# BlackCloud37/rust-raytracer

Hardware: AMD Instinct MI355X
Metric: Msamples/sec (px*spp), scene_500 1200x1200 1000spp (higher is better)
Workload: dtype f64

## Files before the change

### rust-raytracer_amd/csrc/abi.cpp

```cpp
#include <algorithm>
#include <cmath>
#include <cstdlib>
#include <cstring>
#include <functional>
#include <mutex>
#include <new>
#include <string>
#include <vector>

#include "common/grid_shape.h"
#include "common/rng.h"
#include "common/schedule.h"
#include "device/adaptive.h"
#include "device/ao.h"
#include "device/denoise.h"
#include "device/device.h"
#include "host/frame.h"
#include "host/scene.h"
#include "rtamd.h"

using namespace rtamd;

static thread_local std::string g_err;
static Tuning g_tuning;
// ... 951 lines not shown
}

int rt_tonemap_u8(const double* rgb, size_t n_channels, uint8_t* out) {
    return guard([&] {
        REQUIRE((rgb && out) || n_channels == 0, "null argument");
        for (size_t i = 0; i < n_channels; i++) out[i] = tonemap_channel(rgb[i]);
        return (int)RT_OK;
    });
}
int rt_write_png(const char* path, int width, int height, const uint8_t* rgb) {
    return guard([&] {
        REQUIRE(path, "null path");
        write_png(path, width, height, rgb);
        return (int)RT_OK;
    });
}

int rt_debug_rng_device(uint64_t seed, uint64_t pixel, uint64_t sample, int n, uint64_t* out_host) {
    return guard([&] {
        REQUIRE(n > 0 && out_host, "bad argument");
        if (device_count() < 1) throw RtError(RT_ERR_NO_DEVICE, "no HIP device");
        debug_rng_device(seed, pixel, sample, n, out_host);
        return (int)RT_OK;
    });
}
int rt_debug_rng_host(uint64_t seed, uint64_t pixel, uint64_t sample, int n, uint64_t* out_host) {
    return guard([&] {
        REQUIRE(n > 0 && out_host, "bad argument");
        Rng r;
        r.seed_stream(seed, pixel, sample);
        for (int i = 0; i < n; i++) out_host[i] = r.next_u64();
        return (int)RT_OK;
    });
}
int rt_debug_rng_floats(uint64_t seed, uint64_t pixel, uint64_t sample, int n, double lo, double hi, int on_device, double* out_gen,
                        double* out_range) {
    return guard([&] {
        REQUIRE(n > 0 && out_gen && out_range && lo < hi && std::isfinite(hi - lo), "bad argument");
        if (on_device) {
            if (device_count() < 1) throw RtError(RT_ERR_NO_DEVICE, "no HIP device");
            debug_rng_floats_device(seed, pixel, sample, n, lo, hi, out_gen, out_range);
            return (int)RT_OK;
        }
        Rng r;
        r.seed_stream(seed, pixel, sample);
        for (int i = 0; i < n; i++) out_gen[i] = r.gen_f64();
        r.seed_stream(seed, pixel, sample);
        for (int i = 0; i < n; i++) out_range[i] = (lo == -1. && hi == 1.) ? r.gen_range_pm1() : (lo == 0. && hi == 1.) ? r.gen_range_01() : r.gen_range(lo, hi);
        return (int)RT_OK;
    });
}
int rt_debug_math_device(int op, size_t n, const double* a_host, const double* b_host, double* out_host) {
    return guard([&] {
        REQUIRE(n > 0 && a_host && out_host && (op == 0 || op == 2 || op == 3 || (op == 1 && b_host)), "bad argument");
        if (device_count() < 1) throw RtError(RT_ERR_NO_DEVICE, "no HIP device");
        debug_math_device(op, n, a_host, b_host, out_host);
        return (int)RT_OK;
    });
}
int rt_debug_hit_device(const rt_scene* s, int kernel, size_t n, const double* rays_host, double t_min, double t_max, double* out_host) {
    return guard([&] {
        REQUIRE(s && n > 0 && rays_host && out_host && (kernel == 1 || kernel == 2 || kernel == 3 || kernel == 5 || kernel == 6 || kernel == 7), "bad argument");
        if (device_count() < 1) throw RtError(RT_ERR_NO_DEVICE, "no HIP device");
        debug_hit_device(*s, kernel, n, rays_host, t_min, t_max, out_host);
        return (int)RT_OK;
    });
}
static int env_debug(const rt_scene* s, int device, const std::function<void()>& f) {
    return guard([&] {
        REQUIRE(s, "null scene");
        const int n_dev = device_count();
        if (n_dev < 1 || !env_debug_linked()) throw RtError(RT_ERR_NO_DEVICE, "no HIP device");
        REQUIRE(device >= 0 && device < n_dev, "no such device");
        DeviceScope dev_scope(device);
        f();
        return (int)RT_OK;
    });
}
int rt_debug_env_table_device(const rt_scene* s, int device, int* w, int* h, uint32_t* q_host) {
    return env_debug(s, device, [&] { debug_env_table_device(*s, w, h, q_host); });
}
int rt_debug_env_sample_device(const rt_scene* s, int device, size_t n, const double* xi4_host, double* out_host) {
    return env_debug(s, device, [&] {
        REQUIRE(n > 0 && xi4_host && out_host, "bad argument");
        debug_env_eval_device(*s, 0, n, xi4_host, out_host);
    });
}
int rt_debug_env_pdf_device(const rt_scene* s, int device, size_t n, const double* dirs_host, double* pdf_host) {
    return env_debug(s, device, [&] {
        REQUIRE(n > 0 && dirs_host && pdf_host, "bad argument");
        debug_env_eval_device(*s, 1, n, dirs_host, pdf_host);
    });
}
int rt_debug_area_sample_device(const rt_scene* s, int device, size_t n, const double* in_host, double* out_host) {
    return env_debug(s, device, [&] {
        REQUIRE(n > 0 && in_host && out_host, "bad argument");
        if (&rtamd::debug_area_eval_device == nullptr) throw RtError(RT_ERR_NO_DEVICE, "no HIP device");
        debug_area_eval_device(*s, 0, n, in_host, out_host);
    });
}
int rt_debug_area_pdf_device(const rt_scene* s, int device, size_t n, const double* rays_host, double* pdf_host) {
    return env_debug(s, device, [&] {
        REQUIRE(n > 0 && rays_host && pdf_host, "bad argument");
        if (&rtamd::debug_area_eval_device == nullptr) throw RtError(RT_ERR_NO_DEVICE, "no HIP device");
        debug_area_eval_device(*s, 1, n, rays_host, pdf_host);
    });
}
// ... 154 lines not shown
```

### rust-raytracer_amd/csrc/device/kernels.hip

```cpp
#include <hip/hip_runtime.h>

#include <cmath>
#include <cstdio>
#include <chrono>
#include <cstdlib>
#include <cstring>
#include <map>
#include <memory>
#include <mutex>
#include <vector>

#include "../common/flat.h"
#include "../common/grid_shape.h"
#include "../common/detlog.h"
#include "../common/detsin.h"
#include "../common/detuv.h"
#include "../common/rng.h"
#include "../common/schedule.h"
#include "../common/tighten.h"
#include "device.h"

namespace rtamd {

#ifndef PT_BLOCK
// ... 61 lines not shown
DEV double dot(D3 a, D3 b) { return a.x * b.x + a.y * b.y + a.z * b.z; }
DEV double sqlen(D3 a) { return a.x * a.x + a.y * a.y + a.z * a.z; }
DEV D3 cross(D3 a, D3 b) { return mk(a.y * b.z - a.z * b.y, a.z * b.x - a.x * b.z, a.x * b.y - a.y * b.x); }
DEV double comp(D3 a, int i) { return i == 0 ? a.x : (i == 1 ? a.y : a.z); }
DEV D3 unit(D3 a, int* err) {
    double l = sqrt(sqlen(a));
    if (l == 0.) atomicOr(err, 1);
    return divs(a, l);
}
DEV bool near_zero(D3 a) {
    const double S = 1e-8;
    return (fabs(a.x) < S) && (fabs(a.y) < S) && (fabs(a.z) < S);
}
DEV D3 reflect(D3 v, D3 n) { return sub(v, muls(n, 2. * dot(v, n))); }
DEV D3 refract(D3 uv, D3 n, double eta) {
    double cos_theta = fmin(dot(neg(uv), n), 1.0);
    D3 perp = muls(add(uv, muls(n, cos_theta)), eta);
    D3 par = muls(n, -sqrt(fabs(1.0 - sqlen(perp))));
    return add(perp, par);
}
DEV D3 random_in_unit_sphere(Rng& rng) {
    double u, v, r2;
    for (;;) {
        u = rng.gen_range_pm1();
        v = rng.gen_range_pm1();
        r2 = u * u + v * v;
        if (r2 <= 1.) break;
    }
    double q = sqrt(1. - r2);
    return mk(2. * u * q, 2. * v * q, 1. - 2. * r2);
}
DEV D3 random_in_unit_disk(Rng& rng) {
    for (;;) {
        double a = rng.gen_range_pm1();
        double b = rng.gen_range_pm1();
        if (a * a + b * b + 0. * 0. >= 1.) continue;
        return mk(a, b, 0.);
    }
}
DEV D3 xf_point(const double* t, D3 p) {
    return mk(t[0] * p.x + t[1] * p.y + t[2] * p.z + t[3] * 1., t[4] * p.x + t[5] * p.y + t[6] * p.z + t[7] * 1.,
              t[8] * p.x + t[9] * p.y + t[10] * p.z + t[11] * 1.);
}
DEV D3 xf_dir(const double* t, D3 p) {
    return mk(t[0] * p.x + t[1] * p.y + t[2] * p.z + t[3] * 0., t[4] * p.x + t[5] * p.y + t[6] * p.z + t[7] * 0.,
              t[8] * p.x + t[9] * p.y + t[10] * p.z + t[11] * 0.);
}

#define AS_G __attribute__((address_space(1)))
#define AS_L __attribute__((address_space(3)))
typedef unsigned int u32x4 __attribute__((ext_vector_type(4)));
typedef float f32x4 __attribute__((ext_vector_type(4)));
typedef float f32x2 __attribute__((ext_vector_type(2)));
struct Acc {
    const uint2* meta;
    const double2* boxes;
    const double2* spheres;
    const int* sphere_mat;
    const double2* rects;
    const int* rect_mat;
    const uint4* tris;
    const double2* tripre;
    const double2* tripre2;
    const AS_L f32x4* n2_top;
    uint32_t n2_top_count;
    uint32_t n2w_lds;
    const double* xforms;
    const MatDev* mats;
    const TexDev* texs;
    const double* vpos;
    const double* vnrm;
    const uint8_t* texels;
    uint32_t n_nodes;
    const float4* n2;
    const uint2* items2;
    const uint2* inst2;
    uint32_t root2;
    const uint2* lights;
    uint32_t n_lights;
    const MediumDev* media;
    const double* msph;
    const uint32_t* tie_view;
    uint32_t time_lds;
    const uint4* n2q;
    const uint4* n2q_top;
    uint32_t n2q_top_count;
    const uint4* tri32;
    const double* qgrid;
};
template <class P>
DEV Acc make_acc(P hot, const char* gbase, const FlatView& v) {
    Acc a;
    a.meta = (const uint2*)(hot + v.off_meta);
    a.boxes = (const double2*)(hot + v.off_boxes);
    a.spheres = (const double2*)(hot + v.off_spheres);
    a.rects = (const double2*)(hot + v.off_rects);
    a.tris = (const uint4*)(hot + v.off_tris);
    a.tripre = (const double2*)(hot + v.off_tripre);
    a.tripre2 = (const double2*)(hot + v.off_tripre2);
    a.n2_top = nullptr;
    a.n2_top_count = 0;
    a.n2w_lds = 0;
    a.xforms = (const double*)(hot + v.off_xforms);
    a.vpos = (const double*)(gbase + v.off_vpos);
    a.sphere_mat = (const int*)(gbase + v.off_sphere_mat);
    a.rect_mat = (const int*)(gbase + v.off_rect_mat);
    a.mats = (const MatDev*)(gbase + v.off_mats);
    a.texs = (const TexDev*)(gbase + v.off_texs);
    a.vnrm = (const double*)(gbase + v.off_vnrm);
    a.texels = (const uint8_t*)(gbase + v.off_texels);
    a.n_nodes = v.n_nodes;
    a.n2 = (const float4*)(hot + v.off_n2);
    a.items2 = (const uint2*)(hot + v.off_items2);
    a.inst2 = (const uint2*)(hot + v.off_inst2);
    a.root2 = v.root2;
    a.lights = (const uint2*)(gbase + v.off_lights);
    a.n_lights = v.n_lights;
    a.media = (const MediumDev*)(gbase + v.off_media);
    a.msph = (const double*)(gbase + v.off_msph);
    a.tie_view = (const uint32_t*)(gbase + v.off_tie_view);
    a.time_lds = 0u;
    return a;
}

struct CamK {
    D3 origin, llc, horizontal, vertical, u, v;
    double lens_radius;
};
struct RenderK {
    int width, height, max_depth;
    double t_min;
    uint64_t seed;
    int s_begin, s_end;
    int sub_spp, subs_per_tile, n_units;
    int tiles_x, rank, world;
    int tiles_owned;
    int job_units;
    int lvl[5][5];
    int pool_mode;
    const double* sppm_est;
    int n_top;
    int n_topq;
    int coop_pool;
    int coop_stack;
    double time0, time1;
    int time_slots;
    const int* tile_list;
    float box_shrink;
};

DEV bool aabb_hit(const double2* b, D3 o, D3 inv, double t_min, double t_max) {
    double2 v0 = b[0], v1 = b[1], v2 = b[2];
    double mn = t_min, mx = t_max;
    {
        double t0 = (v0.x - o.x) * inv.x, t1 = (v1.y - o.x) * inv.x;
        if (inv.x < 0.0) { double s = t0; t0 = t1; t1 = s; }
        mn = fmax(mn, t0);
        mx = fmin(mx, t1);
    }
    {
        double t0 = (v0.y - o.y) * inv.y, t1 = (v2.x - o.y) * inv.y;
        if (inv.y < 0.0) { double s = t0; t0 = t1; t1 = s; }
        mn = fmax(mn, t0);
        mx = fmin(mx, t1);
    }
    {
        double t0 = (v1.x - o.z) * inv.z, t1 = (v2.y - o.z) * inv.z;
        if (inv.z < 0.0) { double s = t0; t0 = t1; t1 = s; }
        mn = fmax(mn, t0);
        mx = fmin(mx, t1);
    }
    return !(mx <= mn);
}
#ifndef RT_SPHERE_F32_REJECT
#define RT_SPHERE_F32_REJECT 0
#endif
DEV bool sphere_hit(const double2* s, D3 o, D3 d, double a, double t_min, double t_max, double& t_out) {
    double2 c0 = s[0], c1 = s[1];
    D3 oc = mk(o.x - c0.x, o.y - c0.y, o.z - c1.x);
    double radius = c1.y;
    if (RT_SPHERE_F32_REJECT) {
        const float x = (float)oc.x, y = (float)oc.y, z = (float)oc.z, dx = (float)d.x, dy = (float)d.y, dz = (float)d.z, r32 = (float)radius;
        const float hb = __builtin_fmaf(z, dz, __builtin_fmaf(y, dy, x * dx));
        const float a32 = __builtin_fmaf(dz, dz, __builtin_fmaf(dy, dy, dx * dx));
        const float c32 = __builtin_fmaf(z, z, __builtin_fmaf(y, y, x * x)) - r32 * r32;
        const float disc32 = __builtin_fmaf(hb, hb, -(a32 * c32));
        const float m = fmaxf(fmaxf(fabsf(x), fabsf(y)), fabsf(z)) + fabsf(r32), dm = fmaxf(fmaxf(fabsf(dx), fabsf(dy)), fabsf(dz));
        const float bound = 7.62939453125e-06f * (dm * m) * (dm * m);
        if (disc32 < -bound) return false;
    }
    double half_b = dot(oc, d);
    double c = sqlen(oc) - radius * radius;
    double disc = half_b * half_b - a * c;
    if (disc < 0.) return false;
    double sq = sqrt(disc);
    double root = (-half_b - sq) / a;
    if (!(root >= t_min && root <= t_max)) root = (-half_b + sq) / a;
    if (!(root >= t_min && root <= t_max)) return false;
    t_out = root;
    return true;
}
DEV bool rect_hit(const double2* r, int axis, D3 o, D3 d, double t_min, double t_max, double& t_out) {
    double2 r0 = r[0], r1 = r[1], r2 = r[2];
    double t = (r2.x - comp(o, axis)) / comp(d, axis);
    if (t < t_min || t > t_max) return false;
    D3 p = add(o, muls(d, t));
    double a, b;
    if (axis == 2) { a = p.x; b = p.y; }
    else if (axis == 1) { a = p.x; b = p.z; }
    else { a = p.y; b = p.z; }
    if (a < r0.x || a > r1.x || b < r0.y || b > r1.y) return false;
    t_out = t;
    return true;
}
DEV double ray_time(const Acc& A) { return A.time_lds ? *(const AS_L double*)(uintptr_t)(A.time_lds + 8u * threadIdx.x) : 0.; }
DEV D3 msphere_center(const double* q, double time) {
    const D3 c0 = mk(q[0], q[1], q[2]), c1 = mk(q[3], q[4], q[5]);
    return add(c0, muls(sub(c1, c0), (time - q[6]) / (q[7] - q[6])));
}
__device__ __attribute__((noinline)) bool msphere_hit(const double* q, double time, double ox, double oy, double oz, double dx, double dy, double dz, double a,
                                                       double t_min, double t_max, double* t_out) {
    const D3 c = msphere_center(q, time), o = mk(ox, oy, oz), d = mk(dx, dy, dz);
    const D3 oc = sub(o, c);
    const double radius = q[8];
    const double half_b = dot(oc, d);
    const double cc = sqlen(oc) - radius * radius;
    const double disc = half_b * half_b - a * cc;
    if (disc < 0.) return false;
    const double sq = sqrt(disc);
    double root = (-half_b - sq) / a;
    if (!(root >= t_min && root <= t_max)) root = (-half_b + sq) / a;
    if (!(root >= t_min && root <= t_max)) return false;
    *t_out = root;
    return true;
}
DEV int perlin_cell(double fx) {
    const double m = fx - 256. * floor(fx * 0.00390625);
    return (m >= 0. && m < 256.) ? (int)m : 0;
}
__device__ __attribute__((noinline)) double noise_marble(const uint8_t* tab, double scale, double px, double py, double pz) {
    const double* ranvec = (const double*)tab;
    const uint8_t* perm = tab + 768 * sizeof(double);
    double accum_t = 0., weight = 1.;
    double x = px, y = py, z = pz;
    const double NEAR = 33554432.;
    const bool near = (fabs(px) < NEAR) && (fabs(py) < NEAR) && (fabs(pz) < NEAR);
    for (int oct = 0; oct < 7; oct++) {
        const double fx = floor(x), fy = floor(y), fz = floor(z);
        const double u = x - fx, v = y - fy, w = z - fz;
        int i, j, k;
        if (near) {
            i = (int)fx; j = (int)fy; k = (int)fz;
        } else {
// ... 346 lines not shown
    const float tf = fminf(fminf(qx, qy), qz);
    entry = tn;
    float m;
    asm("v_min_f32 %0, %1, %2" : "=v"(m) : "v"(tf), "v"(r.best));
    return !(tn > m) && !(r.tmin > tf);
}
DEV bool box32s(float nx, float ny, float nz, float fx, float fy, float fz, const Ray32& r, float& entry) {
    const float px = __builtin_fmaf(nx, r.ix, -r.cx), qx = __builtin_fmaf(fx, r.ix, -r.cx);
    const float py = __builtin_fmaf(ny, r.iy, -r.cy), qy = __builtin_fmaf(fy, r.iy, -r.cy);
    const float pz = __builtin_fmaf(nz, r.iz, -r.cz), qz = __builtin_fmaf(fz, r.iz, -r.cz);
    const float tn = fmaxf(fmaxf(px, py), pz);
    const float tf = fminf(fminf(qx, qy), qz) * (1.0f + 9.5367431640625e-7f);
    entry = tn;
    return !(tn > tf) && !(tn > r.best) && !(r.tmin > tf);
}
struct SignMasks {
    uint64_t x, y, z;
};
DEV SignMasks sign_masks(const Ray32& r) {
    SignMasks m;
    m.x = __ballot(r.ix < 0.f);
    m.y = __ballot(r.iy < 0.f);
    m.z = __ballot(r.iz < 0.f);
    return m;
}
DEV uint32_t sel32(uint32_t if_clear, uint32_t if_set, uint64_t lane_mask) {
    uint32_t v;
    asm("v_cndmask_b32_e64 %0, %1, %2, %3" : "=v"(v) : "v"(if_clear), "v"(if_set), "s"(lane_mask));
    return v;
}
DEV bool box32(float lox, float loy, float loz, float hix, float hiy, float hiz, const Ray32& r, float& entry) {
    float px = __builtin_fmaf(lox, r.ix, -r.cx), qx = __builtin_fmaf(hix, r.ix, -r.cx);
    float py = __builtin_fmaf(loy, r.iy, -r.cy), qy = __builtin_fmaf(hiy, r.iy, -r.cy);
    float pz = __builtin_fmaf(loz, r.iz, -r.cz), qz = __builtin_fmaf(hiz, r.iz, -r.cz);
    float tn = fmaxf(fmaxf(fminf(px, qx), fminf(py, qy)), fminf(pz, qz));
    float tf = fminf(fminf(fmaxf(px, qx), fmaxf(py, qy)), fmaxf(pz, qz)) * (1.0f + 9.5367431640625e-7f);
    entry = tn;
    return !(tn > tf) && !(tn > r.best) && !(r.tmin > tf);
}

__host__ __device__ inline size_t walk_stack_bytes(uint32_t rows, uint32_t threads) { return (size_t)rows * threads * sizeof(uint32_t); }
__host__ __device__ inline uint32_t coop_stack_rows(const FlatView& v) {
    const uint32_t d = (v.world_depth2 > v.inst_depth2 ? v.world_depth2 : v.inst_depth2) + 2u;
    return d > v.stack2_inline ? d : v.stack2_inline;
}
struct MediaTrack {
    uint32_t lim[2];
    double exitt[2];
    double T[2];
};
DEV double track_bound(const MediaTrack& K, double best) {
    return fmax(best, fmax(K.lim[0] != 0u ? fmin(K.T[0], K.exitt[0]) : 0., K.lim[1] != 0u ? fmin(K.T[1], K.exitt[1]) : 0.));
}
template <int GENERAL, bool DEFER = false, bool TOP = true, bool WIDE = false, class PEND = uint32_t, bool LIMIT = false, bool ENTER = !DEFER, bool TRACK = false, bool RESOLVE = true,
          bool TIEDEF = false>
DEV Hit traverse2(const Acc& A, uint32_t* stk, const int stride, D3 wo, D3 wd, double t_min, double t_max, PEND* pend = nullptr, uint32_t order_limit = 0xFFFFFFFFu,
                  MediaTrack* track = nullptr) {
    D3 o = wo, d = wd;
    Hit h;
    h.t = t_max;
    h.node = -1;
    h.xf = -1;
    h.kp = 0;
    int cur_xf = -1;
    double a = sqlen(d);
    constexpr bool TIE = TIE_RULE && GENERAL != 0 && (!DEFER || TIEDEF) && !LIMIT && !(TRACK && RT_TIE_NOTRACK);
    Ray32 r = make_ray32(o, d, t_min, t_max);
    float best_all32 = r.best;
    if (WIDE) ray32_wide_addr(r, A.n2w_lds);
    int sp = 0;
    const uint32_t spw_step = 4u * (uint32_t)stride;
    uint32_t spw = WIDE ? (uint32_t)(uintptr_t)(AS_L uint32_t*)stk + spw_step : 0u;
    if (WIDE) *(AS_L uint32_t*)stk = REF_DONE;
    uint32_t cur = WIDE ? wide_ref(A.root2) : A.root2;
    for (;;) {
        while ((cur >> REF_TAG_SHIFT) == 0u) {
            PH_EV(10);
#ifdef RTAMD_PHASE_STATS
            if (GENERAL && cur_xf >= 0) PH_EV(15);
#endif
            if (WIDE) {
                const uint32_t axx = cur + r.ax, ayy = cur + r.ay, azz = cur + r.az;
                f32x2 nx, fx, ny, fy, nz, fz, cc;
                asm volatile(
                    "ds_read_b64 %0, %7\n\t"
                    "ds_read_b64 %1, %7 offset:%10\n\t"
                    "ds_read_b64 %2, %8\n\t"
                    "ds_read_b64 %3, %8 offset:%10\n\t"
                    "ds_read_b64 %4, %9\n\t"
                    "ds_read_b64 %5, %9 offset:%10\n\t"
                    "ds_read_b64 %6, %7 offset:24\n\t"
                    "s_waitcnt lgkmcnt(0)"
                    : "=&v"(nx), "=&v"(fx), "=&v"(ny), "=&v"(fy), "=&v"(nz), "=&v"(fz), "=&v"(cc)
                    : "v"(axx), "v"(ayy), "v"(azz), "n"(NODEW_FAR)
                    : "memory");
                float e0, e1;
                const bool h0 = box32w(nx.x, ny.x, nz.x, fx.x, fy.x, fz.x, r, e0);
                const bool h1 = box32w(nx.y, ny.y, nz.y, fx.y, fy.y, fz.y, r, e1);
                const uint32_t c0 = __float_as_uint(cc.x), c1 = __float_as_uint(cc.y);
                if (h0 && h1) {
                    const bool swap = e1 < e0;
                    *(AS_L uint32_t*)(uintptr_t)spw = swap ? c0 : c1;
                    spw += spw_step;
                    cur = swap ? c1 : c0;
                } else if (h0) {
                    cur = c0;
                } else if (h1) {
                    cur = c1;
// ... 1 lines not shown
                    spw -= spw_step;
                    cur = *(const AS_L uint32_t*)(uintptr_t)spw;
                }
                continue;
            }
            f32x4 q0, q1, q2;
            f32x2 q3;
            f32x2 q3m = {0.f, 0.f};
            if (TOP && cur < A.n2_top_count) {
                const AS_L f32x4* p = A.n2_top + NODE2_F4 * cur;
                q0 = p[0]; q1 = p[1]; q2 = p[2]; q3 = *(const AS_L f32x2*)(p + 3);
                if (LIMIT || TRACK) q3m = ((const AS_L f32x2*)(p + 3))[1];
            } else {
                const f32x4* p = (const f32x4*)A.n2 + NODE2_F4 * cur;
                q0 = p[0]; q1 = p[1]; q2 = p[2]; q3 = *(const f32x2*)(p + 3);
                if (LIMIT || TRACK) q3m = ((const f32x2*)(p + 3))[1];
            }
            float e0, e1;
            bool h0 = box32(q0.x, q0.z, q1.x, q1.z, q2.x, q2.z, r, e0);
            bool h1 = box32(q0.y, q0.w, q1.y, q1.w, q2.y, q2.w, r, e1);
            if (LIMIT) {
                h0 = h0 && __float_as_uint(q3m.x) < order_limit;
                h1 = h1 && __float_as_uint(q3m.y) < order_limit;
            }
            if (TRACK) {
                const uint32_t lim = max(track->lim[0], track->lim[1]);
                h0 = h0 && (__float_as_uint(q3m.x) < lim || !(e0 > best_all32));
                h1 = h1 && (__float_as_uint(q3m.y) < lim || !(e1 > best_all32));
            }
            uint32_t c0 = __float_as_uint(q3.x), c1 = __float_as_uint(q3.y);
            if (h0 && h1) {
                bool swap = e1 < e0;
                uint32_t nearc = swap ? c1 : c0, farc = swap ? c0 : c1;
                stk[sp] = farc;
                sp += stride;
                cur = nearc;
            } else if (h0) {
                cur = c0;
            } else if (h1) {
                cur = c1;
            } else if (sp > 0) {
                sp -= stride;
                cur = stk[sp];
            } else {
                cur = REF_DONE;
            }
        }
        if (!WIDE && cur == REF_DONE) break;
        PH_BEGIN(ph_leaf0);
        if (WIDE && cur == REF_DONE) {
        } else if ((cur >> REF_TAG_SHIFT) == 1u) {
            uint32_t first = cur & REF_LEAF_FIRST_MASK, cnt = ((cur >> REF_LEAF_COUNT_SHIFT) & 7u) + 1u;
            uint32_t enter = REF_DONE;
            for (uint32_t i = 0; i < cnt; i++) {
                PH_EV(11);
                uint2 it = A.items2[first + i];
                uint32_t kind = it.x & NK_MASK, pl = it.x >> NK_BITS;
                double t = 0.;
                bool got = false;
                uint32_t cube_side = 0u;
                const double t_far = TRACK ? track_bound(*track, TIE ? h.t * TIE_W : h.t) : (TIE ? h.t * TIE_W : h.t);
                if (LIMIT && it.y >= order_limit) {
                } else if (kind == NK_SPHERE) {
                    got = sphere_hit(A.spheres + 2 * pl, o, d, a, t_min, t_far, t);
                } else if (GENERAL) {
                    if (kind == NK_RECT_YZ || kind == NK_RECT_XZ || kind == NK_RECT_XY) {
                        got = rect_hit(A.rects + 3 * pl, (int)kind - (int)NK_RECT_YZ, o, d, t_min, t_far, t);
                    } else if (GENERAL >= 2 && kind == NK_MSPHERE) {
                        got = msphere_hit(A.msph + 10 * pl, ray_time(A), o.x, o.y, o.z, d.x, d.y, d.z, a, t_min, t_far, &t);
                    } else if (kind == NK_CUBE) {
                        PH_EV(12);
                        got = cube_hit(A.rects + 3 * (pl >> 3), o, d, t_min, t_far, t, cube_side);
                    } else if (kind == NK_TRI) {
                        double b1, b2;
                        got = tri_hit(A.tripre2 + 5 * (first + i), o, d, t_min, t_far, t, b1, b2);
                    } else if (DEFER && kind == NK_INSTANCE) {
                        *pend |= (PEND)1 << pl;
                    } else if (ENTER) {
                        enter = pl;
                    }
                }
                if (TRACK) {
                    if (got) {
                        if (it.y < track->lim[0] && t < track->T[0]) track->T[0] = t;
                        if (it.y < track->lim[1] && t < track->T[1]) track->T[1] = t;
                        if (t < h.t || (t == h.t && (int)it.y > h.node) || !(t == t)) {
                            const bool tied = TIE && h.node >= 0 && t * TIE_W >= h.t;
                            h.t = t;
                            h.node = (int)it.y;
                            h.xf = tied ? (cur_xf ^ TIE_FLAG) : cur_xf;
                            h.kp = it.x + (cube_side << NK_BITS);
                            best_all32 = ray32_best(t);
                        } else if (TIE && !(t > h.t * TIE_W) && (int)it.y < h.node && !tie_flagged(h.xf)) {
                            h.xf ^= TIE_FLAG;
                        }
                        r.best = ray32_best(track_bound(*track, h.t));
                    }
                } else if (got) {
                    if (TIE ? !(t < h.t || (t == h.t && (int)it.y > h.node) || !(t == t)) : !(t < h.t || (int)it.y > h.node || !(t == t))) {
                        if (TIE && (int)it.y < h.node && !tie_flagged(h.xf)) h.xf ^= TIE_FLAG;
                        continue;
                    }
                    const bool tied = TIE && h.node >= 0 && t * TIE_W >= h.t;
                    h.t = t;
                    h.node = (int)it.y;
                    h.xf = tied ? (cur_xf ^ TIE_FLAG) : cur_xf;
                    h.kp = it.x + (cube_side << NK_BITS);
// ... 252 lines not shown
    EnvTab e;
    e.hdr = (const EnvTabHdr*)tab;
    e.rowcum = (const uint64_t*)(tab + sizeof(EnvTabHdr));
    e.cum = e.rowcum + e.hdr->h;
    return e;
}
DEV D3 env_dir(double u, double v, double& st) {
    const double PI = 3.14159265358979323846264338327950288;
    const double theta = PI * v, phi = (2.0 * PI) * u;
    st = det_sin(theta);
    const double ct = det_sin(theta + PI / 2.0), cp = det_sin(phi + PI / 2.0), sp = det_sin(phi);
    return mk(-(cp * st), -ct, sp * st);
}
DEV uint32_t env_search(const uint64_t* __restrict__ p, uint32_t n, uint64_t t) {
    uint32_t lo = 0u, hi = n - 1u;
    while (lo < hi) {
        const uint32_t mid = (lo + hi) >> 1;
        if (p[mid] > t) hi = mid;
        else lo = mid + 1u;
    }
    return lo;
}
__device__ __attribute__((noinline)) D3 env_sample(const char* tab, double x1, double x2, double x3, double x4) {
    const EnvTab e = env_tab(tab);
    const uint32_t W = e.hdr->w, H = e.hdr->h;
    const uint64_t total = e.hdr->total;
    uint64_t t = (uint64_t)(x1 * (double)total);
    if (t > total - 1ull) t = total - 1ull;
    const uint32_t j = env_search(e.rowcum, H, t);
    const uint64_t* row = e.cum + (size_t)j * W;
    const uint64_t row_total = row[W - 1u];
    uint64_t tc = (uint64_t)(x2 * (double)row_total);
    if (tc > row_total - 1ull) tc = row_total - 1ull;
    const uint32_t i = env_search(row, W, tc);
    double st;
    return env_dir(((double)i + x3) / (double)W, ((double)j + x4) / (double)H, st);
}
__device__ __attribute__((noinline)) double env_pdf(const char* tab, D3 d, int* err) {
    const double PI = 3.14159265358979323846264338327950288;
    const EnvTab e = env_tab(tab);
    const uint32_t W = e.hdr->w, H = e.hdr->h;
    const D3 n = unit(d, err);
    double u, v;
    sphere_uv(n, u, v);
    int i = (int)floor((double)W * u), j = (int)floor((double)H * v);
    i = i < 0 ? 0 : (i > (int)W - 1 ? (int)W - 1 : i);
    j = j < 0 ? 0 : (j > (int)H - 1 ? (int)H - 1 : j);
    const double s2 = 1.0 - n.y * n.y;
    if (!(s2 > 0.)) return 0.;
    const uint64_t* row = e.cum + (size_t)j * W;
    const uint64_t q = row[i] - (i > 0 ? row[i - 1] : 0ull);
    return ((((double)q / (double)e.hdr->total) * (double)W) * (double)H) / (((2.0 * PI) * PI) * sqrt(s2));
}
template <int GENERAL, bool ALL_UV = false>
DEV Rec materialize(const Acc& A, const Hit& h, D3 wo, D3 wd, int* err) {
    Rec rec;
    uint32_t kind = h.kp & NK_MASK, pl = h.kp >> NK_BITS;
    D3 o = wo, d = wd;
    if (GENERAL == 3 && h.xf >= 0) {
        chain_ray(A, (uint32_t)h.xf, CHAIN_ALL, o, d);
    } else if (GENERAL && h.xf >= 0) {
        const double* Minv = A.xforms + 32 * h.xf;
        o = xf_point(Minv, wo);
        d = xf_dir(Minv, wd);
    }
    D3 outward;
    rec.u = 0.;
    rec.v = 0.;
    bool want_uv = false;
    if (GENERAL == 0 || kind == NK_SPHERE) {
        double2 c0 = A.spheres[2 * pl], c1 = A.spheres[2 * pl + 1];
        rec.mat = A.sphere_mat[pl];
        D3 p = add(o, muls(d, h.t));
        outward = divs(sub(p, mk(c0.x, c0.y, c1.x)), c1.y);
        want_uv = ALL_UV || A.texs[A.mats[rec.mat].tex].type == 2;
        if (want_uv) sphere_uv(outward, rec.u, rec.v);
    } else if (GENERAL >= 2 && kind == NK_MSPHERE) {
        const double* q = A.msph + 10 * pl;
        rec.mat = (int)q[9];
        D3 p = add(o, muls(d, h.t));
        outward = divs(sub(p, msphere_center(q, ray_time(A))), q[8]);
        want_uv = ALL_UV || A.texs[A.mats[rec.mat].tex].type == 2;
        if (want_uv) sphere_uv(outward, rec.u, rec.v);
    } else if (GENERAL && kind == NK_MEDIUM_END) {
        rec.mat = A.media[pl].mat;
        outward = mk(1., 0., 0.);
    } else if (GENERAL && kind != NK_TRI) {
        int axis = (int)kind - (int)NK_RECT_YZ;
        double2 r0, r1;
        if (kind == NK_CUBE) {
            const uint32_t side = pl & 7u;
            pl >>= 3;
            const double2 c0 = A.rects[3 * pl], c1 = A.rects[3 * pl + 1], c2 = A.rects[3 * pl + 2];
            axis = side < 2u ? 2 : (side < 4u ? 1 : 0);
            if (axis == 2) { r0 = c0; r1.x = c1.y; r1.y = c2.x; }
            else if (axis == 1) { r0.x = c0.x; r0.y = c1.x; r1.x = c1.y; r1.y = c2.y; }
            else { r0.x = c0.y; r0.y = c1.x; r1.x = c2.x; r1.y = c2.y; }
        } else {
            r0 = A.rects[3 * pl];
            r1 = A.rects[3 * pl + 1];
        }
        rec.mat = A.rect_mat[pl];
        outward = mk(axis == 0 ? 1. : 0., axis == 1 ? 1. : 0., axis == 2 ? 1. : 0.);
        if (ALL_UV || A.texs[A.mats[rec.mat].tex].type == 2) {
            D3 p = add(o, muls(d, h.t));
            double a, b;
            if (axis == 2) { a = p.x; b = p.y; }
            else if (axis == 1) { a = p.x; b = p.z; }
            else { a = p.y; b = p.z; }
            rec.u = (a - r0.x) / (r1.x - r0.x);
            rec.v = (b - r0.y) / (r1.y - r0.y);
        }
    } else if (GENERAL) {
        uint4 tr = A.tris[pl];
        rec.mat = (int)tr.w;
        double t, b1 = 0., b2 = 0.;
        tri_hit(A.tripre + 5 * pl, o, d, -INFINITY, INFINITY, t, b1, b2);
        double b0 = 1.0 - b1 - b2;
        D3 na = ld3(A.vnrm, tr.x), nb = ld3(A.vnrm, tr.y), nc = ld3(A.vnrm, tr.z);
        outward = unit(add(add(muls(na, b0), muls(nb, b1)), muls(nc, b2)), err);
    } else {
        outward = mk(0., 0., 0.);
        rec.mat = 0;
    }
// ... 592 lines not shown
                job_n = min(L[4], L[5 + 1] - job_blk0);
                job_k = 0;
            }
            job_lvl |= (int)(list_cursor << 8);
        }
        if (job_k < job_n) {
            const int tile = job_image_tile(cfg, job_tile);
            u.tx = tile % cfg[CFG_TILES_X];
            u.ty = tile / cfg[CFG_TILES_X];
            const int sub_i = job_blk0 + job_k;
            const AS_L int* L = cfg + CFG_LVL + 5 * (job_lvl & 0xff);
            u.s0 = L[2] + (sub_i - L[1]) * L[3];
            const int s1 = min(u.s0 + L[3], L[5 + 2]);
            u.pool = (s1 - u.s0) * TILE_PIX;
            u.cur_slot = r_head + r_cnt;
            if (u.cur_slot >= ring_units) u.cur_slot -= ring_units;
            r_cnt++;
            if (lane == 0) {
                AS_L uint32_t* m = rmeta + 4 * u.cur_slot;
                m[0] = (uint32_t)job_tile;
                m[1] = (uint32_t)sub_i;
                m[2] = (uint32_t)(s1 - u.s0) | (job_k == 0 ? 0x100u : 0u) | (job_k + 1 == job_n ? 0x200u : 0u);
                const int w_in = min(TILE_W, cfg[CFG_WIDTH] - u.tx * TILE_W), h_in = min(TILE_H, cfg[CFG_HEIGHT] - u.ty * TILE_H);
                __hip_atomic_store(&m[3], (uint32_t)((s1 - u.s0) * w_in * h_in), __ATOMIC_RELAXED, __HIP_MEMORY_SCOPE_WORKGROUP);
            }
            job_k++;
        }
    }
    u.finished = (u.pool == 0 && !more_jobs && job_k >= job_n && r_cnt == 0) ? 1 : 0;
    if (lane == 0) {
        wst[0] = (uint32_t)r_head; wst[1] = (uint32_t)r_cnt; wst[2] = (uint32_t)job_tile; wst[3] = (uint32_t)job_blk0;
        wst[4] = (uint32_t)job_n; wst[5] = (uint32_t)job_k; wst[6] = more_jobs ? 1u : 0u; wst[7] = (uint32_t)job_lvl;
    }
    return u;
}

#ifndef RT_TIGHTEN_BOXES
#define RT_TIGHTEN_BOXES 1
#endif
static constexpr int INTEG_BG = 4;
static constexpr int INTEG_ENV = 8;
static constexpr int INTEG_AREA = 16;
template <bool LDS, int GENERAL, int ACCEL, int INTEG, bool MEDIA = false, bool POOL = false>
__global__ void __launch_bounds__(PT_BLOCK) pt_kernel(FlatView sv, CamK cam, RenderK rk, double* __restrict__ ring, double* accum,
                                                      unsigned int* tickets, unsigned int* __restrict__ counter, int* __restrict__ err) {
    extern __shared__ __attribute__((aligned(16))) char smem[];
#ifdef RT_TAIL_STATS
    const unsigned long long tail_entry = __builtin_amdgcn_s_memrealtime();
#endif
    const uint32_t st_begin = (ACCEL == 2) ? sv.stage2_begin : 0u;
    const uint32_t st_end = (ACCEL == 2) ? sv.stage2_end : sv.stage_bytes;
    uint32_t staged = 0;
    Acc A;
    if (LDS && ACCEL == 2) {
        const uint32_t lo_bytes = sv.off_n2 - st_begin;
        {
            const uint4* src = (const uint4*)(sv.base + st_begin);
            uint4* dst = (uint4*)smem;
            for (uint32_t i = threadIdx.x; i < lo_bytes / 16; i += blockDim.x) dst[i] = src[i];
        }
        char* n2w = smem + lo_bytes;
        stage_nodew(sv, n2w, rk.box_shrink);
        staged = lo_bytes + nodew_bytes(sv.n_nodes2);
        __syncthreads();
        A = make_acc(smem - st_begin, sv.base, sv);
        A.n2 = nullptr;
        A.n2w_lds = (uint32_t)(uintptr_t)(AS_L char*)n2w;
        if (MEDIA) {
            A.meta = (const uint2*)(sv.base + sv.off_meta);
            A.boxes = (const double2*)(sv.base + sv.off_boxes);
        }
    } else if (LDS) {
        const uint4* src = (const uint4*)(sv.base + st_begin);
        uint4* dst = (uint4*)smem;
        for (uint32_t i = threadIdx.x; i < (st_end - st_begin) / 16; i += blockDim.x) dst[i] = src[i];
        staged = st_end - st_begin;
        __syncthreads();
        A = make_acc(smem - st_begin, sv.base, sv);
    } else {
        A = make_acc(sv.base, sv.base, sv);
        if (ACCEL == 2 && rk.n_top > 0) {
            const uint4* src = (const uint4*)(sv.base + sv.off_n2);
            uint4* dst = (uint4*)smem;
            for (uint32_t i = threadIdx.x; i < (uint32_t)rk.n_top * NODE2_F4; i += blockDim.x) dst[i] = src[i];
            __syncthreads();
            A.n2_top = (const AS_L f32x4*)smem;
            A.n2_top_count = (uint32_t)rk.n_top;
            staged = (uint32_t)rk.n_top * (uint32_t)sizeof(Node2);
        }
    }
    const char* area_env = nullptr;
    if ((INTEG & INTEG_AREA) && sv.off_env != 0u && ((const EnvTabHdr*)(sv.base + sv.total_bytes))->total != 0ull) area_env = sv.base + sv.total_bytes;
    uint32_t* stk = (uint32_t*)(smem + staged) + threadIdx.x;
    const int stk_stride = (int)blockDim.x;
    const int lane = threadIdx.x & 63;
    const uint64_t lanemask_lt = (1ull << lane) - 1ull;
    const int wave = threadIdx.x >> 6;
    uint32_t* book = (uint32_t*)(smem + staged + walk_stack_bytes((ACCEL == 2) ? sv.stack2 : 0u, PT_BLOCK));
    uint32_t* rmeta = book + (size_t)wave * RING_UNITS * 4;
    uint32_t* wst = book + (size_t)(PT_BLOCK / 64) * RING_UNITS * 4 + (size_t)wave * 8;
    int* cfg = (int*)(book + (size_t)(PT_BLOCK / 64) * (RING_UNITS * 4 + 8));
    if (lane < 8) wst[lane] = (lane == 6) ? 1u : 0u;
    if (POOL && lane < RING_UNITS * 4) rmeta[lane] = 0u;
    if (threadIdx.x == 0) {
        cfg[CFG_N_JOBS] = rk.n_units; cfg[CFG_TILES_OWNED] = rk.tiles_owned; cfg[CFG_JOB_UNITS] = rk.job_units;
        cfg[CFG_SUBS_PER_TILE] = rk.subs_per_tile; cfg[CFG_WORLD] = rk.world; cfg[CFG_RANK] = rk.rank; cfg[CFG_TILES_X] = rk.tiles_x;
        cfg[CFG_S_BEGIN] = rk.s_begin; cfg[CFG_S_END] = rk.s_end; cfg[CFG_SUB_SPP] = rk.sub_spp; cfg[CFG_WIDTH] = rk.width;
        cfg[CFG_HEIGHT] = rk.height;
        cfg[CFG_RING_UNITS] = RING_UNITS;
// ... 93 lines not shown
                                const double2 e0 = wbatch[pix], e1 = wbatch[TILE_PIX + pix], e2 = wbatch[2 * TILE_PIX + pix], e3 = wbatch[3 * TILE_PIX + pix];
                                o = mk(e0.x, e0.y, e1.x);
                                d = mk(e1.y, e2.x, e2.y);
                                rng.s = (uint64_t)__double_as_longlong(e3.x);
                                beta = mk(1., 1., 1.);
                                L = mk(0., 0., 0.);
                                depth = rk.max_depth;
                                pix_id = y * rk.width + x;
                                out_slot = ((uint32_t)cur_slot * (uint32_t)UNIT_SPP + (uint32_t)b) * (uint32_t)TILE_PIX + (uint32_t)pix;
                                alive = true;
                            }
                        }
                        b += 1;
                        due = true;
                        if ((b << 6) >= next_end) break;
                    }
                } else {
                    if (!alive && k < pool) {
                        PH_EV(16);
                        int pix = k & (TILE_PIX - 1), s = s0 + (k >> 6);
                        int x = tx * TILE_W + (pix & (TILE_W - 1)), y = ty * TILE_H + (pix >> 3);
                        if (x < rk.width && y < rk.height) {
                            rng.seed_stream(rk.seed, (uint64_t)y * (uint64_t)rk.width + (uint64_t)x, (uint64_t)s);
                            double u = ((double)x + rng.gen_f64()) / (double)(rk.width - 1);
                            double v = ((double)y + rng.gen_f64()) / (double)(rk.height - 1);
                            double st = 1.0 - v;
                            D3 rd = muls(random_in_unit_disk(rng), cam.lens_radius);
                            if (GENERAL >= 2 && rk.time1 > rk.time0) {
                                const double tm = rng.gen_range(rk.time0, rk.time1);
                                if (A.time_lds) *(AS_L double*)(uintptr_t)(A.time_lds + 8u * threadIdx.x) = tm;
                            } else if (GENERAL >= 2 && A.time_lds) {
                                *(AS_L double*)(uintptr_t)(A.time_lds + 8u * threadIdx.x) = rk.time0;
                            }
                            D3 offset = add(muls(cam.u, rd.x), muls(cam.v, rd.y));
                            o = add(cam.origin, offset);
                            d = sub(sub(add(add(cam.llc, muls(cam.horizontal, u)), muls(cam.vertical, st)), cam.origin), offset);
                            beta = mk(1., 1., 1.);
                            L = mk(0., 0., 0.);
                            depth = rk.max_depth;
                            pix_id = y * rk.width + x;
                            out_slot = ((uint32_t)cur_slot * (uint32_t)UNIT_SPP + (uint32_t)(k >> 6)) * (uint32_t)TILE_PIX + (uint32_t)pix;
                            alive = true;
                        }
                    }
                }
                next = next_end;
            }
            PH_END(0, ph_it0);
            if (__ballot(alive) == 0ull && next >= pool && finished) break;
            if (alive) {
                PH_EV(13);
                PH_BEGIN(ph_t0);
                Hit h = (ACCEL == 2) ? (MEDIA ? traverse2_media<GENERAL, !LDS, LDS>(A, sv.n_media, stk, stk_stride, o, d, rk.t_min, rng)
                                              : traverse2<GENERAL, false, !LDS, LDS>(A, stk, stk_stride, o, d, rk.t_min, INFINITY))
                                     : traverse<GENERAL, MEDIA>(A, o, d, rk.t_min, INFINITY, &rng);
                PH_END(1, ph_t0);
                PH_BEGIN(ph_p0);
                bool done = true;
                if (h.node >= 0 && depth > 0) {
                    depth -= 1;
                    PH_BEGIN(ph_m0);
                    const Rec rec = materialize<GENERAL>(A, h, o, d, err);
                    PH_END(2, ph_m0);
                    constexpr bool SEG_IN_PLACE = !(GENERAL == 1 && !LDS && ACCEL == 2 && INTEG == INTEG_BG && MEDIA) &&
                                                  !(GENERAL == 3 && LDS && ACCEL == 1 && INTEG == (INTEG_BG | 1));
                    if (SEG_IN_PLACE) o = rec.p;
                    D3 emitted, att, ndir = d;
                    D3& nd = SEG_IN_PLACE ? d : ndir;
                    bool diffuse, scattered;
                    PH_BEGIN(ph_s0);
                    if constexpr (GENERAL == 0) {
                        const auto add_emitted = [&](const D3& le) {
                            L = add(L, elemul(beta, le));
                            asm volatile("" : "+v"(L.x), "+v"(L.y), "+v"(L.z));
                        };
                        scattered = shade<GENERAL>(A, rec, d, rng, emitted, att, nd, diffuse, err, add_emitted);
                    } else {
                        scattered = shade<GENERAL>(A, rec, d, rng, emitted, att, nd, diffuse, err);
                        L = add(L, elemul(beta, emitted));
                    }
                    PH_END(3, ph_s0);
                    if (scattered) {
                        if ((INTEG & 3) == 2 && diffuse) {
                            const double* e = rk.sppm_est + 6 * (size_t)pix_id;
                            L = add(L, elemul(beta, mk(e[0], e[1], e[2])));
                            L = add(L, elemul(beta, mk(e[3], e[4], e[5])));
                        } else if ((INTEG & 3) == 1 && diffuse) {
                            PH_EV(14);
                            if (INTEG & INTEG_AREA) done = !mixture_step_area(A, sv.base + sv.off_area, area_env, rec, rng, att, beta, nd, err);
                            else if (INTEG & INTEG_ENV) done = !mixture_step_env(A, sv.base + sv.total_bytes, rec, rng, att, beta, nd, err);
                            else done = !mixture_step(A, rec, rng, att, beta, nd, err);
                        } else {
                            beta = elemul(beta, att);
                            done = false;
                        }
                        if (!SEG_IN_PLACE && !done) {
                            o = rec.p;
                            d = ndir;
                        }
                    }
                } else if ((INTEG & INTEG_BG) && h.node < 0 && (!(INTEG & INTEG_AREA) || sv.off_bg != 0u)) {
                    L = add(L, elemul(beta, background_radiance<GENERAL>((const BgDev*)(sv.base + sv.off_bg), A.texs, A.texels, d, err)));
                }
                if (done) {
                    double* dst = wring + 3 * (size_t)out_slot;
                    dst[0] = L.x;
                    dst[1] = L.y;
                    dst[2] = L.z;
                    atomicSub(rmeta + 4 * (out_slot >> 9) + 3, 1u);
                    alive = false;
                }
                PH_END(8, ph_p0);
            }
        }
    }
// ... 979 lines not shown
#endif
}

__global__ void finalize_kernel(const double* __restrict__ accum, double* __restrict__ tiles, int64_t n_pix, int spp, int width,
                                int height, int tiles_x, int rank, int world) {
    int64_t i = (int64_t)blockIdx.x * blockDim.x + threadIdx.x;
    if (i >= n_pix) return;
    int64_t lt = i >> 6;
    int pix = (int)(i & 63);
    int64_t tile = lt * world + rank;
    int x = (int)(tile % tiles_x) * TILE_W + (pix & 7), y = (int)(tile / tiles_x) * TILE_H + (pix >> 3);
    bool inside = x < width && y < height;
    double n = (double)spp;
    tiles[3 * i] = inside ? accum[3 * i] / n : 0.;
    tiles[3 * i + 1] = inside ? accum[3 * i + 1] / n : 0.;
    tiles[3 * i + 2] = inside ? accum[3 * i + 2] / n : 0.;
}
__global__ void assemble_kernel(const double* __restrict__ gathered, int64_t stride_tiles, double* __restrict__ frame, int width,
                                int height, int tiles_x, int world) {
    int64_t i = (int64_t)blockIdx.x * blockDim.x + threadIdx.x;
    int64_t n = (int64_t)width * height;
    if (i >= n) return;
    int x = (int)(i % width), y = (int)(i / width);
    int64_t tile = (int64_t)(y >> 3) * tiles_x + (x >> 3);
    int r = (int)(tile % world);
    int64_t lt = tile / world;
    int pix = ((y & 7) << 3) | (x & 7);
    const double* src = gathered + (((int64_t)r * stride_tiles + lt) * TILE_PIX + pix) * 3;
    frame[3 * i] = src[0];
    frame[3 * i + 1] = src[1];
    frame[3 * i + 2] = src[2];
}

#include "wavefront.inc"
#include "sppm.inc"

__global__ void rng_kernel(uint64_t seed, uint64_t pixel, uint64_t sample, int n, uint64_t* out) {
    if (threadIdx.x != 0 || blockIdx.x != 0) return;
    Rng r;
    r.seed_stream(seed, pixel, sample);
    for (int i = 0; i < n; i++) out[i] = r.next_u64();
}
__global__ void rng_floats_kernel(uint64_t seed, uint64_t pixel, uint64_t sample, int n, double lo, double hi, double* out) {
    if (threadIdx.x != 0 || blockIdx.x != 0) return;
    Rng r;
    r.seed_stream(seed, pixel, sample);
    for (int i = 0; i < n; i++) out[i] = r.gen_f64();
    r.seed_stream(seed, pixel, sample);
    for (int i = 0; i < n; i++) out[n + i] = (lo == -1. && hi == 1.) ? r.gen_range_pm1() : (lo == 0. && hi == 1.) ? r.gen_range_01() : r.gen_range(lo, hi);
}
__global__ void math_kernel(int op, size_t n, const double* a, const double* b, double* out) {
    size_t i = (size_t)blockIdx.x * blockDim.x + threadIdx.x;
    if (i >= n) return;
    out[i] = (op == 0) ? sqrt(a[i]) : (op == 2) ? det_ln(a[i]) : (op == 3) ? det_sin(a[i]) : a[i] / b[i];
}
DEV void hit_row(double* q, const Hit& h, const Rec& rec) {
    q[0] = 1.;
    q[1] = h.t;
    q[2] = rec.p.x; q[3] = rec.p.y; q[4] = rec.p.z;
    q[5] = rec.normal.x; q[6] = rec.normal.y; q[7] = rec.normal.z;
    q[8] = rec.front_face ? 1. : 0.;
    q[9] = rec.u; q[10] = rec.v;
    q[11] = (double)h.node;
}
__global__ void hit_kernel(FlatView sv, int accel, float box_shrink, size_t n, const double* rays, double t_min, double t_max, double* out, int* err) {
    extern __shared__ __attribute__((aligned(16))) char smem[];
    size_t i = (size_t)blockIdx.x * blockDim.x + threadIdx.x;
    Acc A = make_acc(sv.base, sv.base, sv);
    uint32_t stack_at = 0;
    if (accel == 3) {
        stage_nodew(sv, smem, box_shrink);
        __syncthreads();
        A.n2w_lds = (uint32_t)(uintptr_t)(AS_L char*)smem;
        stack_at = nodew_bytes(sv.n_nodes2);
    }
    if (i >= n) return;
    D3 o = mk(rays[6 * i], rays[6 * i + 1], rays[6 * i + 2]), d = mk(rays[6 * i + 3], rays[6 * i + 4], rays[6 * i + 5]);
    uint32_t* stk = (uint32_t*)(smem + stack_at) + threadIdx.x;
    Hit h;
    if (accel == 5 || accel == 6) {
        uint64_t pend = 0ull;
        h = traverse2<true, true, false, false, uint64_t, false, true, false, false, true>(A, stk, (int)blockDim.x, o, d, t_min, t_max, &pend);
        if (tie_flagged(h.xf)) {
            h = tie_resolve<1>(A, o, d, t_min, t_max, h);
            pend = 0ull;
        }
        bool tied = false;
        ServeCtx X;
        X.n2q = (const AS_G u32x4*)(sv.base + sv.off_n2q);
        X.tri32 = (const AS_G u32x4*)(sv.base + sv.off_tri32);
        X.n2q_top = nullptr;
        X.n_topq = 0u;
        while (pend != 0ull) {
            const uint32_t ni = (uint32_t)(__ffsll((long long)pend) - 1);
            pend &= pend - 1ull;
            const uint2 in = A.inst2[ni];
            const double* Minv = A.xforms + 32 * in.x;
            const D3 oo = xf_point(Minv, o), dd = xf_dir(Minv, d);
            double ht = h.t;
            int hnode = h.node, sp = 0;
            uint32_t hkp = 0u, cur = in.y;
            if (accel == 5) {
                const double a = sqlen(dd);
                Ray32 r = make_ray32(oo, dd, t_min, h.t);
                while (cur != REF_DONE) blas_pass<true>(A, true, stk, (int)blockDim.x, oo, dd, a, t_min, r, ht, hnode, hkp, cur, sp, err, tied);
            } else {
                const double* g = (const double*)(sv.base + sv.off_qgrid) + 8 * ni;
// ... 1491 lines not shown
```

Baseline: 3127.

## Pre-resolve leaf items to LDS sphere addresses and use fast f64 sqrt

While staging the BVH into LDS for the sphere-only path, leaf item words are rewritten to hold direct LDS byte addresses of sphere records. The leaf loop can then load sphere data without kind decoding or index arithmetic, and materialize recovers the primitive index from that address. Sphere intersection also uses a custom rsq-plus-Newton sqrt that falls back to the library sqrt whenever any lane in the wave has an out-of-range input. This trades extra staging work and a wave-wide ballot for fewer ALU ops per leaf, and relies on the refined sqrt matching the library result bit for bit.

```diff
diff --git a/rust-raytracer_amd/csrc/abi.cpp b/rust-raytracer_amd/csrc/abi.cpp
--- a/rust-raytracer_amd/csrc/abi.cpp
+++ b/rust-raytracer_amd/csrc/abi.cpp
@@ -1027,7 +1027,7 @@
 }
 int rt_debug_math_device(int op, size_t n, const double* a_host, const double* b_host, double* out_host) {
     return guard([&] {
-        REQUIRE(n > 0 && a_host && out_host && (op == 0 || op == 2 || op == 3 || (op == 1 && b_host)), "bad argument");
+        REQUIRE(n > 0 && a_host && out_host && (op == 0 || op == 2 || op == 3 || op == 4 || (op == 1 && b_host)), "bad argument");
         if (device_count() < 1) throw RtError(RT_ERR_NO_DEVICE, "no HIP device");
         debug_math_device(op, n, a_host, b_host, out_host);
         return (int)RT_OK;
diff --git a/rust-raytracer_amd/csrc/device/kernels.hip b/rust-raytracer_amd/csrc/device/kernels.hip
--- a/rust-raytracer_amd/csrc/device/kernels.hip
+++ b/rust-raytracer_amd/csrc/device/kernels.hip
@@ -137,6 +137,8 @@
 typedef unsigned int u32x4 __attribute__((ext_vector_type(4)));
 typedef float f32x4 __attribute__((ext_vector_type(4)));
 typedef float f32x2 __attribute__((ext_vector_type(2)));
+typedef unsigned int u32x2 __attribute__((ext_vector_type(2)));
+typedef double f64x2 __attribute__((ext_vector_type(2)));
 struct Acc {
     const uint2* meta;
     const double2* boxes;
@@ -173,6 +175,7 @@
     const uint4* tri32;
     const double* qgrid;
 };
+DEV uint32_t lds_addr(const void* p) { return (uint32_t)(uintptr_t)(const AS_L char*)(const char*)p; }
 template <class P>
 DEV Acc make_acc(P hot, const char* gbase, const FlatView& v) {
     Acc a;
@@ -257,11 +260,24 @@
     }
     return !(mx <= mn);
 }
+DEV double sqrt_hot(double x) {
+    const uint32_t hi = (uint32_t)((uint64_t)__double_as_longlong(x) >> 32);
+    if (__ballot(hi - 0x10000000u >= 0x7FF00000u - 0x10000000u) != 0ull) return sqrt(x);
+    const double y = __builtin_amdgcn_rsq(x);
+    double g = x * y, h = y * 0.5;
+    const double r = __builtin_fma(-h, g, 0.5);
+    g = __builtin_fma(g, r, g);
+    h = __builtin_fma(h, r, h);
+    g = __builtin_fma(__builtin_fma(-g, g, x), h, g);
+    g = __builtin_fma(__builtin_fma(-g, g, x), h, g);
+    return g;
+}
 #ifndef RT_SPHERE_F32_REJECT
 #define RT_SPHERE_F32_REJECT 0
 #endif
-DEV bool sphere_hit(const double2* s, D3 o, D3 d, double a, double t_min, double t_max, double& t_out) {
-    double2 c0 = s[0], c1 = s[1];
+template <bool HOT = false, class SP, class F>
+DEV bool sphere_root(SP s, D3 o, D3 d, double a, double t_min, double t_max, F&& accept) {
+    const auto c0 = s[0], c1 = s[1];
     D3 oc = mk(o.x - c0.x, o.y - c0.y, o.z - c1.x);
     double radius = c1.y;
     if (RT_SPHERE_F32_REJECT) {
@@ -278,12 +294,15 @@
     double c = sqlen(oc) - radius * radius;
     double disc = half_b * half_b - a * c;
     if (disc < 0.) return false;
-    double sq = sqrt(disc);
+    double sq = HOT ? sqrt_hot(disc) : sqrt(disc);
     double root = (-half_b - sq) / a;
     if (!(root >= t_min && root <= t_max)) root = (-half_b + sq) / a;
     if (!(root >= t_min && root <= t_max)) return false;
-    t_out = root;
+    accept(root);
     return true;
+}
+DEV bool sphere_hit(const double2* s, D3 o, D3 d, double a, double t_min, double t_max, double& t_out) {
+    return sphere_root(s, o, d, a, t_min, t_max, [&](double root) __attribute__((always_inline)) { t_out = root; });
 }
 DEV bool rect_hit(const double2* r, int axis, D3 o, D3 d, double t_min, double t_max, double& t_out) {
     double2 r0 = r[0], r1 = r[1], r2 = r[2];
@@ -736,8 +755,28 @@
 DEV double track_bound(const MediaTrack& K, double best) {
     return fmax(best, fmax(K.lim[0] != 0u ? fmin(K.T[0], K.exitt[0]) : 0., K.lim[1] != 0u ? fmin(K.T[1], K.exitt[1]) : 0.));
 }
+#ifndef ITEM_SQRT_HOT
+#define ITEM_SQRT_HOT true
+#endif
+DEV void leaf_items_addr(uint32_t ia, uint32_t cnt, D3 o, D3 d, double a, double t_min, Hit& h, Ray32& r) {
+    const uint32_t ie = ia + 8u * cnt;
+    do {
+        PH_EV(11);
+        const u32x2 it = *(const AS_L u32x2*)(uintptr_t)ia;
+        ia += 8u;
+        asm("" : "+v"(ia));
+        sphere_root<ITEM_SQRT_HOT>((const AS_L f64x2*)(uintptr_t)it.x, o, d, a, t_min, h.t, [&](double t) __attribute__((always_inline)) {
+            if ((t < h.t) | ((int)it.y > h.node) | !(t == t)) {
+                h.t = t;
+                h.node = (int)it.y;
+                h.kp = it.x;
+                r.best = ray32_best(t);
+            }
+        });
+    } while (ia != ie);
+}
 template <int GENERAL, bool DEFER = false, bool TOP = true, bool WIDE = false, class PEND = uint32_t, bool LIMIT = false, bool ENTER = !DEFER, bool TRACK = false, bool RESOLVE = true,
-          bool TIEDEF = false>
+          bool TIEDEF = false, bool ITEMA = false>
 DEV Hit traverse2(const Acc& A, uint32_t* stk, const int stride, D3 wo, D3 wd, double t_min, double t_max, PEND* pend = nullptr, uint32_t order_limit = 0xFFFFFFFFu,
                   MediaTrack* track = nullptr) {
     D3 o = wo, d = wd;
@@ -845,7 +884,9 @@
         } else if ((cur >> REF_TAG_SHIFT) == 1u) {
             uint32_t first = cur & REF_LEAF_FIRST_MASK, cnt = ((cur >> REF_LEAF_COUNT_SHIFT) & 7u) + 1u;
             uint32_t enter = REF_DONE;
-            for (uint32_t i = 0; i < cnt; i++) {
+            static_assert(!ITEMA || (WIDE && GENERAL == 0 && !DEFER && !LIMIT && !TRACK), "ITEMA: the sphere-only LDS walk");
+            if constexpr (ITEMA) leaf_items_addr(lds_addr(A.items2) + 8u * first, cnt, o, d, a, t_min, h, r);
+            for (uint32_t i = 0; !ITEMA && i < cnt; i++) {
                 PH_EV(11);
                 uint2 it = A.items2[first + i];
                 uint32_t kind = it.x & NK_MASK, pl = it.x >> NK_BITS;
@@ -1204,10 +1245,10 @@
     const uint64_t q = row[i] - (i > 0 ? row[i - 1] : 0ull);
     return ((((double)q / (double)e.hdr->total) * (double)W) * (double)H) / (((2.0 * PI) * PI) * sqrt(s2));
 }
-template <int GENERAL, bool ALL_UV = false>
+template <int GENERAL, bool ALL_UV = false, bool ITEMA = false>
 DEV Rec materialize(const Acc& A, const Hit& h, D3 wo, D3 wd, int* err) {
     Rec rec;
-    uint32_t kind = h.kp & NK_MASK, pl = h.kp >> NK_BITS;
+    uint32_t kind = h.kp & NK_MASK, pl = ITEMA ? (h.kp - lds_addr(A.spheres)) >> 5 : h.kp >> NK_BITS;
     D3 o = wo, d = wd;
     if (GENERAL == 3 && h.xf >= 0) {
         chain_ray(A, (uint32_t)h.xf, CHAIN_ALL, o, d);
@@ -1221,7 +1262,17 @@
     rec.v = 0.;
     bool want_uv = false;
     if (GENERAL == 0 || kind == NK_SPHERE) {
-        double2 c0 = A.spheres[2 * pl], c1 = A.spheres[2 * pl + 1];
+        double2 c0, c1;
+        if constexpr (ITEMA) {
+            static_assert(!ITEMA || GENERAL == 0, "ITEMA: the sphere-only LDS walk");
+            const AS_L f64x2* s = (const AS_L f64x2*)(uintptr_t)h.kp;
+            const f64x2 s0 = s[0], s1 = s[1];
+            c0 = make_double2(s0.x, s0.y);
+            c1 = make_double2(s1.x, s1.y);
+        } else {
+            c0 = A.spheres[2 * pl];
+            c1 = A.spheres[2 * pl + 1];
+        }
         rec.mat = A.sphere_mat[pl];
         D3 p = add(o, muls(d, h.t));
         outward = divs(sub(p, mk(c0.x, c0.y, c1.x)), c1.y);
@@ -1920,9 +1971,23 @@
     const uint32_t st_end = (ACCEL == 2) ? sv.stage2_end : sv.stage_bytes;
     uint32_t staged = 0;
     Acc A;
+    constexpr bool ITEMA = LDS && GENERAL == 0 && ACCEL == 2 && !MEDIA;
     if (LDS && ACCEL == 2) {
         const uint32_t lo_bytes = sv.off_n2 - st_begin;
-        {
+        if constexpr (ITEMA) {
+            const uint32_t sph_lds = lds_addr(smem) + (sv.off_spheres - st_begin);
+            const uint32_t it0 = (sv.off_items2 - st_begin) / 16, it1 = (sv.off_inst2 - st_begin) / 16;
+            const uint4* src = (const uint4*)(sv.base + st_begin);
+            uint4* dst = (uint4*)smem;
+            for (uint32_t i = threadIdx.x; i < lo_bytes / 16; i += blockDim.x) {
+                uint4 w = src[i];
+                if (i >= it0 && i < it1) {
+                    w.x = sph_lds + ((w.x >> NK_BITS) << 5);
+                    w.z = sph_lds + ((w.z >> NK_BITS) << 5);
+                }
+                dst[i] = w;
+            }
+        } else {
             const uint4* src = (const uint4*)(sv.base + st_begin);
             uint4* dst = (uint4*)smem;
             for (uint32_t i = threadIdx.x; i < lo_bytes / 16; i += blockDim.x) dst[i] = src[i];
@@ -2122,7 +2187,7 @@
                 PH_EV(13);
                 PH_BEGIN(ph_t0);
                 Hit h = (ACCEL == 2) ? (MEDIA ? traverse2_media<GENERAL, !LDS, LDS>(A, sv.n_media, stk, stk_stride, o, d, rk.t_min, rng)
-                                              : traverse2<GENERAL, false, !LDS, LDS>(A, stk, stk_stride, o, d, rk.t_min, INFINITY))
+                                              : traverse2<GENERAL, false, !LDS, LDS, uint32_t, false, true, false, true, false, ITEMA>(A, stk, stk_stride, o, d, rk.t_min, INFINITY))
                                      : traverse<GENERAL, MEDIA>(A, o, d, rk.t_min, INFINITY, &rng);
                 PH_END(1, ph_t0);
                 PH_BEGIN(ph_p0);
@@ -2130,7 +2195,7 @@
                 if (h.node >= 0 && depth > 0) {
                     depth -= 1;
                     PH_BEGIN(ph_m0);
-                    const Rec rec = materialize<GENERAL>(A, h, o, d, err);
+                    const Rec rec = materialize<GENERAL, false, ITEMA>(A, h, o, d, err);
                     PH_END(2, ph_m0);
                     constexpr bool SEG_IN_PLACE = !(GENERAL == 1 && !LDS && ACCEL == 2 && INTEG == INTEG_BG && MEDIA) &&
                                                   !(GENERAL == 3 && LDS && ACCEL == 1 && INTEG == (INTEG_BG | 1));
@@ -3216,7 +3281,7 @@
 __global__ void math_kernel(int op, size_t n, const double* a, const double* b, double* out) {
     size_t i = (size_t)blockIdx.x * blockDim.x + threadIdx.x;
     if (i >= n) return;
-    out[i] = (op == 0) ? sqrt(a[i]) : (op == 2) ? det_ln(a[i]) : (op == 3) ? det_sin(a[i]) : a[i] / b[i];
+    out[i] = (op == 0) ? sqrt(a[i]) : (op == 2) ? det_ln(a[i]) : (op == 3) ? det_sin(a[i]) : (op == 4) ? sqrt_hot(a[i]) : a[i] / b[i];
 }
 DEV void hit_row(double* q, const Hit& h, const Rec& rec) {
     q[0] = 1.;
```

Result: faster. 3222, median of 6 (+3.0%).
